# tensor4all/tensor4all-rs

Hardware: AMD Instinct MI355X
Metric: TCI2 full-sweep GF/s (d=30, chi=256 fp64) (higher is better)
Workload: dtype f64

## Files before the change

tensor4all-rs_amd/csrc/kernels.hpp:

```cpp
#pragma once

#include <hip/hip_runtime.h>

#include <cstddef>
#include <cstdint>

#include "../../include/t4a_testfunctions.h"

namespace t4a {

struct RrluWorkspace;

struct RrluPlan {
    int W = 1;
    int T = 256;
    int cpw = 0;
    int Mld = 0;
    size_t lds_bytes = 0;
};

RrluPlan rrlu_make_plan(int M, int N, int num_cus);

struct RrluArgs {
    const double* A;
// ... 160 lines not shown
size_t rrlu_xcd_cols_bytes(const RrluXcdPlan& plan, int M);
struct RrluXcdGroupArgs {
    RrluXcdArgs p[8];
};
void rrlu_xcd2_launch(const RrluXcdPlan& plan, const RrluXcdArgs& args, hipStream_t stream);
void rrlu_xcd2m_launch(const RrluXcdPlan& plan, const RrluXcdArgs& args, hipStream_t stream);
void rrlu_xcd2_group_launch(const RrluXcdPlan& plan, const RrluXcdGroupArgs& args, bool tie_row_major, hipStream_t stream);
bool rrlu_wg_make_plan(int M, int N, RrluXcdPlan* out, int spec_blocks = 0);
void rrlu_wg_launch(const RrluXcdPlan& plan, const RrluXcdArgs& args, hipStream_t stream);
void rrlu_wg_group_launch(const RrluXcdPlan& plan, const RrluXcdGroupArgs& args, bool tie_row_major, hipStream_t stream);
bool rrlu_w1_make_plan(int M, int N, RrluXcdPlan* out, int spec_blocks = 0);
void rrlu_w1_launch(const RrluXcdPlan& plan, const RrluXcdArgs& args, hipStream_t stream);
void rrlu_w1_group_launch(const RrluXcdPlan& plan, const RrluXcdGroupArgs& args, bool tie_row_major, hipStream_t stream);

void pi_eval_launch(const FnDevice& fn, const uint64_t* rowacc, int M, const uint64_t* colacc, int N, double* out,
                    int ld, bool transpose_out, unsigned long long* max_abs_bits, hipStream_t stream);
struct PiJob {
    const uint64_t* rowacc;
    const uint64_t* colacc;
    double* out;
    unsigned long long* max_abs_bits;
    int M, N, ld, pad_;
};
void pi_eval_batched_launch(const FnDevice& fn, const PiJob* d_jobs, int n_jobs, int max_M, int max_N, hipStream_t stream);
struct PackJob {
    const double* src;
    double* core;
    const int* info;
    int ld, L, S, R, last, pad_;
};
struct LuProblem;
constexpr int FILL_SMALL_MAX_N = 32, FILL_SMALL_MAX_RHS = 64;
void fill_small_launch(const FnDevice& fn, const PiJob* d_pis, const LuProblem* d_lups, const PackJob* d_packs, int n_jobs, int last_site,
                       hipStream_t stream);
void stage_copy_launch(const uint64_t* pinned_src, uint64_t* dst, size_t count, hipStream_t stream);
void absmax_launch(const double* data, size_t count, unsigned long long* max_abs_bits, hipStream_t stream);

constexpr int CHAIN_MAX_SET = 1024;
struct ChainTab {
    uint64_t* code;
    uint64_t* acc;
    int* cnt;
};
struct ChainCommon {
    ChainTab I, J, HI, HJ;
    ChainTab mI, mJ;
    int cap, K;
// ... 130 lines not shown

struct LuProblem {
    double* A; int lda; int n;
    int* piv;
    int* info;
    double* B; int ldb; int nrhs;
    const unsigned long long* pmax_bits;
};
void lu_batched_launch(const LuProblem* d_problems, int n_problems, int max_n, hipStream_t stream);
inline TrsmProblem lu_trsm_problem(const LuProblem& lp, bool lower, const int* skip_flag = nullptr)
{
    TrsmProblem t{};
    t.T = lp.A;
    t.ldt = lp.lda;
    t.n = lp.n;
    t.B = lp.B;
    t.ldb = lp.ldb;
    t.nrhs = lp.nrhs;
    t.lower = t.unit_diag = lower ? 1 : 0;
    t.skip_flag = skip_flag;
    return t;
}
constexpr int LU_MAX_PANEL_STEPS = 128;
bool lu_forward_blocked_launch(const LuProblem* d_problems, int n_problems, int max_n, int max_nrhs, hipStream_t stream, int avoid_xcc = -1,
                               unsigned* tickets = nullptr);
bool lu_solve_blocked_launch(const LuProblem* d_problems, int n_problems, int max_n, int max_nrhs, hipStream_t stream, int avoid_xcc = -1,
                             unsigned* tickets = nullptr);

void gather_launch(const double* in, int ldi, const int* rows, int nrows, const int* cols, int ncols, double* out,
                   int ldo, hipStream_t stream);
void scatter_rows_launch(const double* in, int ldi, const int* rows, int nrows, int ncols, double* out, int ldo,
                         hipStream_t stream);
void scatter_cols_launch(const double* in, int ldi, int nrows, const int* cols, int ncols, double* out, int ldo,
                         hipStream_t stream);
void fill_launch(double* p, size_t count, double value, hipStream_t stream);
void seq_matmul_launch(const double* A, int lda, const double* B, int ldb, double* C, int ldc, size_t M, size_t N, size_t K,
                       hipStream_t stream);
void set_identity_launch(double* p, int m, int n, int ld, hipStream_t stream);

struct TtCoreDesc { const double* data; int l, d, r; };
void tt_evaluate_launch(const TtCoreDesc* d_cores, int n_sites, int max_bond, const uint32_t* d_idx, int n_pts,
                        double* d_out, hipStream_t stream);


void core_reshape_launch(const double* in, int L, int S, int R, int mode, double* out, hipStream_t stream);
constexpr int PERMUTE_MAX_RANK = 16;
void permute_launch(const double* in, const size_t* dims, const size_t* perm, int rank, double* out, hipStream_t stream);
void tt_sum_launch(const TtCoreDesc* d_cores, int n_sites, int max_bond, double* d_out, hipStream_t stream);
enum : int {
    TT_SCALE_NONE = 0,
// ... 218 lines not shown
```

tensor4all-rs_amd/csrc/kernels_dense.hip:

```cpp
#include "kernels.hpp"

#include <algorithm>
#include <atomic>
#include <map>
#include <mutex>
#include <utility>
#include "common.hpp"

#include <cstdlib>

namespace t4a {

namespace {

typedef double double4_t __attribute__((ext_vector_type(4)));

constexpr int GBM = 64, GBK = 32, GPAD = 4;

template <int BN>
__global__ void __launch_bounds__(256) gemm_kernel(GemmDesc d)
{
    extern __shared__ __attribute__((aligned(16))) char gemm_smem[];
    typedef double TileA[GBK][GBM + GPAD];
    typedef double TileB[GBK][BN + GPAD];
// ... 625 lines not shown
#pragma unroll
    for (int r = 0; r < RP; ++r) {
        const int i = tid + 256 * r;
        if (i > J && i < m) {
            const double l = a[r][J] / piv;
            a[r][J] = l;
#pragma unroll
            for (int c = J + 1; c < NB; ++c) {
                const double prod = l * U[c];
                a[r][c] = a[r][c] - prod;
            }
        }
    }
}

template <int NB, int RP, int... Js>
__device__ __forceinline__ void lu_panel_columns(double (&a)[RP][NB], const PanelShared& sh, const LuProblem& pr, int kb, int m, int w, int tid,
                                                 int& first_bad, std::integer_sequence<int, Js...>)
{
    (lu_panel_column<NB, RP, Js>(a, sh, pr, kb, m, w, tid, first_bad), ...);
}

template <int NB, int RP>
__global__ void __launch_bounds__(256) lu_panel_kernel(const LuProblem* problems, int kb)
{
    __shared__ double U[2 * NB], V[2 * NB];
    __shared__ double red_v[8];
    __shared__ int red_i[8];
    const LuProblem pr = problems[blockIdx.x];
    const int n = pr.n;
    const int tid = threadIdx.x;
    if (kb == 0) {
        if (pr.pmax_bits) {
            const double pmax = __longlong_as_double((long long)*pr.pmax_bits);
            if (pmax < 2.220446049250313e-16) {
                if (tid == 0) pr.info[0] = -1;
                return;
            }
        }
        if (tid == 0) pr.info[0] = 0;
    } else if (pr.info[0] == -1) {
        return;
    }
    if (kb >= n) return;
    const int m = n - kb, w = (n - kb) < NB ? (n - kb) : NB;
    double* A = pr.A;
    const int lda = pr.lda;
    double a[RP][NB];
#pragma unroll
    for (int r = 0; r < RP; ++r) {
        const int i = tid + 256 * r;
#pragma unroll
        for (int c = 0; c < NB; ++c) a[r][c] = (i < m && c < w) ? A[(size_t)(kb + c) * lda + kb + i] : 0.0;
    }
    int first_bad = 0;
    PanelShared sh{U, V, red_v, red_i};
    lu_panel_columns<NB, RP>(a, sh, pr, kb, m, w, tid, first_bad, std::make_integer_sequence<int, NB>{});
    if (tid == 0 && first_bad != 0 && pr.info[0] == 0) pr.info[0] = first_bad;
#pragma unroll
    for (int r = 0; r < RP; ++r) {
        const int i = tid + 256 * r;
#pragma unroll
        for (int c = 0; c < NB; ++c)
            if (i < m && c < w) A[(size_t)(kb + c) * lda + kb + i] = a[r][c];
    }
}

__global__ void __launch_bounds__(256) lu_update_kernel(const LuProblem* problems, int kb, int nb, int tiles, int n_problems, int avoid_xcc,
                                                        unsigned* ticket, int a_only)
{
    extern __shared__ __attribute__((aligned(16))) char smem_raw[];
    __shared__ int s_item;
    if (avoid_xcc >= 0) {
        unsigned xcc;
        asm volatile("s_getreg_b32 %0, hwreg(HW_REG_XCC_ID)" : "=s"(xcc));
        if ((int)(xcc & 0xF) == avoid_xcc) return;
    }
    const int total_items = tiles * n_problems;
    bool first = true;
    for (;;) {
    __syncthreads();
    if (threadIdx.x == 0) s_item = ticket ? (int)atomicAdd(ticket, 1u) : (first ? (int)blockIdx.x : total_items);
    __syncthreads();
    first = false;
    const int item = s_item;
    if (item >= total_items) break;
    const LuProblem pr = problems[item / tiles];
    const int n = pr.n;
    if (kb >= n || pr.info[0] == -1) continue;
    const int ta = (n + nb - 1) / nb;
    const int nrhs = pr.B ? pr.nrhs : 0;
    const int t = item % tiles;
    const bool in_a = t < ta;
    const int c0 = in_a ? t * nb : (t - ta) * nb;
    if (!in_a && (a_only || c0 >= nrhs)) continue;
    if (in_a && c0 == kb) continue;
    const int m = n - kb, w = (n - kb) < nb ? (n - kb) : nb;
    const int lim = in_a ? n : nrhs;
    const int tc = (lim - c0) < nb ? (lim - c0) : nb;
    const bool left = in_a && c0 < kb;
// ... 104 lines not shown
{
    constexpr int ctrl = Q | (Q << 2) | (Q << 4) | (Q << 6);
    const long long b = __double_as_longlong(v);
    const int lo = __builtin_amdgcn_update_dpp(0, (int)(b & 0xFFFFFFFFll), ctrl, 0xF, 0xF, true);
    const int hi = __builtin_amdgcn_update_dpp(0, (int)(b >> 32), ctrl, 0xF, 0xF, true);
    return __longlong_as_double(((long long)hi << 32) | (unsigned int)lo);
}
template <int KK, bool LOWER> __device__ __forceinline__ void solve_block_step(double (&b)[4], const double (&dr)[SVB][4], const double (&rdr)[SVB], int g)
{
    constexpr int go = KK >> 2, to = KK & 3;
    double xk = quad_bcast_f64<go>(b[to]);
    if (!LOWER) xk = xk * rdr[KK];
    if (g == go) b[to] = xk;
#pragma unroll
    for (int t = 0; t < 4; ++t) b[t] = __builtin_fma(-dr[KK][t], xk, b[t]);
}
template <bool LOWER, int... KKs>
__device__ __forceinline__ void solve_block_steps(double (&b)[4], const double (&dr)[SVB][4], const double (&rdr)[SVB], int g, std::integer_sequence<int, KKs...>)
{
    if constexpr (LOWER) (solve_block_step<KKs, true>(b, dr, rdr, g), ...);
    else (solve_block_step<SVB - 1 - KKs, false>(b, dr, rdr, g), ...);
}

__global__ void __launch_bounds__(256) __attribute__((amdgpu_waves_per_eu(1, 1))) lu_solve_kernel(const LuProblem* problems, int cw, int n_problems, int chunks, int avoid_xcc, unsigned* ticket)
{
    extern __shared__ __attribute__((aligned(16))) char smem_raw[];
    __shared__ int s_item;
    if (avoid_xcc >= 0) {
        unsigned xcc;
        asm volatile("s_getreg_b32 %0, hwreg(HW_REG_XCC_ID)" : "=s"(xcc));
        if ((int)(xcc & 0xF) == avoid_xcc) return;
    }
    const int tid = threadIdx.x;
    const int lane = tid & 63, wave = tid >> 6;
    const int lr = lane & 15, lk = lane >> 4;
    const int cl = lane >> 2, g = lane & 3;
    const int total_items = chunks * n_problems;
    bool first = true;
    for (;;) {
        __syncthreads();
        if (tid == 0) s_item = ticket ? (int)atomicAdd(ticket, 1u) : (first ? (int)blockIdx.x : total_items);
        __syncthreads();
        first = false;
        const int item = s_item;
        if (item >= total_items) break;
        const LuProblem pr = problems[item / chunks];
        const int n = pr.n;
        const int c0 = (item % chunks) * cw;
        if (n <= 0 || !pr.B || c0 >= pr.nrhs || pr.info[0] == -1) continue;
        const int cwr = (pr.nrhs - c0) < cw ? (pr.nrhs - c0) : cw;
        const int ld = n | 1;
        double* Bs = reinterpret_cast<double*>(smem_raw);
        double* D = Bs + (size_t)ld * cw + ((ld * cw) & 1);
        double* rd = D + SVB * SVB;
        unsigned short* perm_s = reinterpret_cast<unsigned short*>(rd + SVB);
// ... 431 lines not shown
            hipLaunchKernelGGL(trsm_left_mfma_kernel, grid, dim3(256), lds, stream, d_problems, cw);
            return;
        }
    }
    int cw = (int)((128 * 1024) / ((size_t)max_n * 8));
    if (cw > 32) cw = 32;
    const long long total_cols = (long long)n_problems * max_nrhs;
    while (cw > 4 && total_cols / cw < 2048) cw /= 2;
    if (cw < 1) cw = 1;
    const size_t lds = (size_t)max_n * cw * 8;
    if (lds > 160 * 1024)
        throw Error(T4A_GPU_NOT_IMPLEMENTED, "triangular solve: systems with more than 20480 rows are not supported");
    dim3 grid((max_nrhs + cw - 1) / cw, n_problems);
    hipLaunchKernelGGL(trsm_left_kernel, grid, dim3(256), lds, stream, d_problems, cw);
}

void lu_batched_launch(const LuProblem* d_problems, int n_problems, int max_n, hipStream_t stream)
{
    if (n_problems <= 0) return;
    int T = max_n >= 128 ? 1024 : (max_n >= 32 ? 256 : 64);
    hipLaunchKernelGGL(lu_kernel, dim3(n_problems), dim3(T), 0, stream, d_problems);
}

bool lu_forward_blocked_launch(const LuProblem* d_problems, int n_problems, int max_n, int max_nrhs, hipStream_t stream, int avoid_xcc,
                               unsigned* tickets)
{
    if (n_problems <= 0 || max_n <= 0) return true;
    int nb;
    if (max_n <= 256) nb = 32;
    else if (max_n <= 512) nb = 16;
    else if (max_n <= 1024) nb = 8;
    else return false;
    static std::atomic<bool> attr_set{false};
    if (!attr_set) {
        (void)hipFuncSetAttribute(reinterpret_cast<const void*>(&lu_update_kernel),
                                  hipFuncAttributeMaxDynamicSharedMemorySize, 144 * 1024);
        (void)hipGetLastError();
        attr_set = true;
    }
    const int ldp = max_n | 1;
    const size_t lds_update = (size_t)ldp * nb * 8 * 2;
    const int tiles = (max_n + nb - 1) / nb + (max_nrhs + nb - 1) / nb + 1;
    for (int kb = 0; kb < max_n; kb += nb) {
        if (nb == 32) hipLaunchKernelGGL((lu_panel_kernel<32, 1>), dim3(n_problems), dim3(256), 0, stream, d_problems, kb);
        else if (nb == 16) hipLaunchKernelGGL((lu_panel_kernel<16, 2>), dim3(n_problems), dim3(256), 0, stream, d_problems, kb);
        else hipLaunchKernelGGL((lu_panel_kernel<8, 4>), dim3(n_problems), dim3(256), 0, stream, d_problems, kb);
        const int items = tiles * n_problems;
        unsigned* tk = tickets ? tickets + kb / nb : nullptr;
        const int grid = tk ? items + items / 7 + 8 : items;
        hipLaunchKernelGGL(lu_update_kernel, dim3(grid), dim3(256), lds_update, stream, d_problems, kb, nb, tiles, n_problems,
                           tk ? avoid_xcc : -1, tk, 0);
    }
    return true;
}

bool lu_solve_blocked_launch(const LuProblem* d_problems, int n_problems, int max_n, int max_nrhs, hipStream_t stream, int avoid_xcc,
                             unsigned* tickets)
{
    if (n_problems <= 0 || max_n <= 0) return true;
    if (max_n < 32 || max_n > 16 * 4 * SV_MAXS || max_nrhs < 16) return false;
    int nb;
    if (max_n <= 256) nb = 32;
    else nb = 16;
    static std::once_flag attr_once;
    std::call_once(attr_once, [] {
        (void)hipFuncSetAttribute(reinterpret_cast<const void*>(&lu_update_kernel), hipFuncAttributeMaxDynamicSharedMemorySize, 144 * 1024);
        (void)hipFuncSetAttribute(reinterpret_cast<const void*>(&lu_solve_kernel), hipFuncAttributeMaxDynamicSharedMemorySize, 160 * 1024);
        (void)hipGetLastError();
    });
    const int ldp = max_n | 1;
    const size_t lds_update = (size_t)ldp * nb * 8 * 2;
    const int tiles = (max_n + nb - 1) / nb;
    for (int kb = 0; kb < max_n; kb += nb) {
        if (nb == 32) hipLaunchKernelGGL((lu_panel_kernel<32, 1>), dim3(n_problems), dim3(256), 0, stream, d_problems, kb);
        else hipLaunchKernelGGL((lu_panel_kernel<16, 2>), dim3(n_problems), dim3(256), 0, stream, d_problems, kb);
        const int items = tiles * n_problems;
        unsigned* tk = tickets ? tickets + kb / nb : nullptr;
        const int grid = tk ? items + items / 7 + 8 : items;
        hipLaunchKernelGGL(lu_update_kernel, dim3(grid), dim3(256), lds_update, stream, d_problems, kb, nb, tiles, n_problems,
                           tk ? avoid_xcc : -1, tk, 1);
    }
    const size_t extra = (size_t)SVB * (SVB + 1) * 8 + SVB * 8 + 2 * (size_t)((max_n + 3) & ~3) * 2 + 64;
    int cw = 64;
    while (cw > 16 && (size_t)(max_n | 1) * cw * 8 + extra > 156 * 1024) cw -= 16;
    if (cw == 48) cw = 32;
    while (cw > 16 && max_nrhs <= cw / 2) cw /= 2;
    const size_t lds = (size_t)(max_n | 1) * cw * 8 + extra;
    const int chunks = (max_nrhs + cw - 1) / cw;
    const int items = chunks * n_problems;
    unsigned* tk = tickets ? tickets + (LU_MAX_PANEL_STEPS - 1) : nullptr;
    const int grid = tk ? items + items / 7 + 8 : items;
    hipLaunchKernelGGL(lu_solve_kernel, dim3(grid), dim3(256), lds, stream, d_problems, cw, n_problems, chunks, tk ? avoid_xcc : -1, tk);
    return true;
}

void tt_evaluate_launch(const TtCoreDesc* d_cores, int n_sites, int max_bond, const uint32_t* d_idx, int n_pts,
                        double* d_out, hipStream_t stream)
{
    if (n_pts <= 0) return;
    int blocks = n_pts < 4096 ? n_pts : 4096;
    const size_t lds = (size_t)2 * (max_bond > 0 ? max_bond : 1) * 8;
    hipLaunchKernelGGL(tt_eval_kernel, dim3(blocks), dim3(256), lds, stream, d_cores, n_sites, max_bond, d_idx, n_pts,
                       d_out);
}

}
```

tensor4all-rs_amd/csrc/kernels_pi.hip:

```cpp
#include "kernels.hpp"

namespace t4a {

namespace {

__device__ __forceinline__ void wave_absmax_commit(double av, unsigned long long* max_abs_bits)
{
#pragma unroll
    for (int off = 32; off >= 1; off >>= 1) {
        const double o = __shfl_xor(av, off);
        if (o > av) av = o;
    }
    if ((threadIdx.x & 63) == 0 && av > 0.0 && max_abs_bits)
        atomicMax(max_abs_bits, (unsigned long long)__double_as_longlong(av));
}

__global__ void __launch_bounds__(256) pi_eval_kernel(FnDevice fn, const uint64_t* __restrict__ rowacc, int M,
                                                      const uint64_t* __restrict__ colacc, int N,
                                                      double* __restrict__ out, int ld, int transpose_out,
                                                      unsigned long long* max_abs_bits)
{
    double av = 0.0;
    const int i = blockIdx.x * blockDim.x + threadIdx.x;
    uint64_t racc[T4A_FN_MAX_ACC] = {0, 0, 0, 0};
    if (i < M)
        for (int k = 0; k < fn.n_acc; ++k) racc[k] = rowacc[(size_t)i * fn.n_acc + k];
    for (int j = blockIdx.y; j < N; j += gridDim.y) {
        if (i < M) {
            uint64_t acc[T4A_FN_MAX_ACC] = {0, 0, 0, 0};
            for (int k = 0; k < fn.n_acc; ++k) acc[k] = racc[k] + colacc[(size_t)j * fn.n_acc + k];
            const double v = t4a_fn_value(fn.fid, acc, fn.params);
            if (transpose_out)
                out[(size_t)i * ld + j] = v;
            else
                out[(size_t)j * ld + i] = v;
            const double a = sqrt(v * v);
            if (a > av) av = a;
        }
    }
    wave_absmax_commit(av, max_abs_bits);
}

__global__ void __launch_bounds__(256) pi_eval_batched_kernel(FnDevice fn, const PiJob* __restrict__ jobs)
{
    const PiJob jb = jobs[blockIdx.z];
    double av = 0.0;
    const int i = blockIdx.x * blockDim.x + threadIdx.x;
    if (blockIdx.x * (int)blockDim.x >= jb.M) return;
    uint64_t racc[T4A_FN_MAX_ACC] = {0, 0, 0, 0};
    if (i < jb.M)
        for (int k = 0; k < fn.n_acc; ++k) racc[k] = jb.rowacc[(size_t)i * fn.n_acc + k];
    for (int j = blockIdx.y; j < jb.N; j += gridDim.y) {
        if (i < jb.M) {
            uint64_t acc[T4A_FN_MAX_ACC] = {0, 0, 0, 0};
            for (int k = 0; k < fn.n_acc; ++k) acc[k] = racc[k] + jb.colacc[(size_t)j * fn.n_acc + k];
            const double v = t4a_fn_value(fn.fid, acc, fn.params);
            jb.out[(size_t)j * jb.ld + i] = v;
            const double a = sqrt(v * v);
            if (a > av) av = a;
        }
    }
    wave_absmax_commit(av, jb.max_abs_bits);
}

__global__ void __launch_bounds__(256) absmax_kernel(const double* __restrict__ data, size_t count,
                                                     unsigned long long* max_abs_bits)
{
    double av = 0.0;
    for (size_t i = (size_t)blockIdx.x * blockDim.x + threadIdx.x; i < count; i += (size_t)gridDim.x * blockDim.x) {
        const double v = data[i];
        const double a = sqrt(v * v);
        if (a > av) av = a;
    }
    wave_absmax_commit(av, max_abs_bits);
}

__global__ void __launch_bounds__(256) stage_copy_kernel(const uint64_t* __restrict__ src, uint64_t* __restrict__ dst, size_t count)
{
    for (size_t i = (size_t)blockIdx.x * blockDim.x + threadIdx.x; i < count; i += (size_t)gridDim.x * blockDim.x) dst[i] = src[i];
}

}

void stage_copy_launch(const uint64_t* pinned_src, uint64_t* dst, size_t count, hipStream_t stream)
{
    if (count == 0) return;
    size_t blocks = (count + 255) / 256;
    if (blocks > 64) blocks = 64;
    hipLaunchKernelGGL(stage_copy_kernel, dim3((unsigned)blocks), dim3(256), 0, stream, pinned_src, dst, count);
}

void pi_eval_launch(const FnDevice& fn, const uint64_t* rowacc, int M, const uint64_t* colacc, int N, double* out,
                    int ld, bool transpose_out, unsigned long long* max_abs_bits, hipStream_t stream)
{
    if (M <= 0 || N <= 0) return;
    dim3 block(256);
    int gy = N < 2048 ? N : 2048;
    dim3 grid((M + 255) / 256, gy);
    hipLaunchKernelGGL(pi_eval_kernel, grid, block, 0, stream, fn, rowacc, M, colacc, N, out, ld,
                       transpose_out ? 1 : 0, max_abs_bits);
}

void pi_eval_batched_launch(const FnDevice& fn, const PiJob* d_jobs, int n_jobs, int max_M, int max_N, hipStream_t stream)
{
    if (n_jobs <= 0 || max_M <= 0 || max_N <= 0) return;
    const int gy = max_N < 512 ? max_N : 512;
    dim3 grid((max_M + 255) / 256, gy, n_jobs);
    hipLaunchKernelGGL(pi_eval_batched_kernel, grid, dim3(256), 0, stream, fn, d_jobs);
}

namespace {

struct FillSmallArgs {
    FnDevice fn;
    const PiJob* pis;
    const LuProblem* lups;
    const PackJob* packs;
    int n_jobs, last_site;
};

__global__ void __launch_bounds__(256) fill_small_kernel(FillSmallArgs a)
{
    __shared__ double As[FILL_SMALL_MAX_N * FILL_SMALL_MAX_N];
    __shared__ double Bs[FILL_SMALL_MAX_N * FILL_SMALL_MAX_RHS];
    __shared__ double red_v[4];
    __shared__ int red_i[4];
    __shared__ int piv_s, info_s;
    __shared__ double pivval_s;
    const int k = blockIdx.x, tid = threadIdx.x, T = blockDim.x, lane = tid & 63, wave = tid >> 6;
    if (k >= a.n_jobs) return;
// ... 167 lines not shown
```

tensor4all-rs_amd/csrc/tci2.hpp:

```cpp
#pragma once

#include <cstring>
#include <memory>
#include <vector>

#include "engine.hpp"
#include "fnsource.hpp"
#include "matrix_source.hpp"
#include "stdrng.hpp"
#include "pishard.hpp"
#include "rook.hpp"
#include "tt.hpp"

namespace t4a {

struct TCI2Options {
    double tolerance = 1e-8;
    size_t max_iter = 20;
    size_t max_bond_dim = 0;
    int pivot_search = 0;
    bool normalize_error = true;
    size_t verbosity = 0;
    size_t max_nglobal_pivot = 5;
    size_t nsearch = 5;
// ... 14 lines not shown
};

struct FillZero {
    double* ptr;
    size_t count;
};
struct FillOps {
    void* flags;
    size_t flag_bytes;
    void* stage_dev;
    const void* stage_host;
    size_t stage_bytes;
    const PiJob* pis;
    const LuProblem* lups;
    const TrsmProblem* trs;
    const PackJob* packs;
    unsigned* tickets;
    const int* info_dev;
    int* info_host;
    size_t info_bytes;
    FnDevice fn;
    int n_pi, max_M, max_N;
    int n_lu, max_n, max_nrhs;
    int avoid_xcc;
    unsigned pack_gx, pack_gy;
    int n_site_jobs, last_site;
    int small;
};
static_assert(sizeof(FillOps) == 13 * 8 + sizeof(FnDevice) + 12 * 4 && sizeof(FnDevice) == 8 + 8 * T4A_FN_MAX_PARAMS, "no padding: compared bytewise");
struct FillRecords {
    std::vector<FillZero> zeros;
    FillOps ops{};
    bool operator==(const FillRecords& o) const
    {
        return zeros.size() == o.zeros.size() && std::memcmp(&ops, &o.ops, sizeof(FillOps)) == 0 &&
               (zeros.empty() || std::memcmp(zeros.data(), o.zeros.data(), zeros.size() * sizeof(FillZero)) == 0);
    }
};
struct FillOptions {
    bool async = false;
    bool trust_cache = false;
    bool no_main_sync = false;
};

class Tci2 {
    pool::IdleScope idle_scope_;
public:
    explicit Tci2(const std::vector<size_t>& local_dims);
    ~Tci2();

    void set_builtin(int fid, int n_acc, const double* params, const uint64_t* weights);
    void set_callback(t4a_gpu_batch_eval_fn cb, void* ctx);
// ... 119 lines not shown
        size_t bond = 0;
        bool cols = false;
        IndexSet set;
        std::vector<uint64_t> acc;
    };
    SidePrep prep_;
    struct Prefetch {
        bool wanted = false;
        size_t bond = 0;
        bool cols = false;
        const IndexSet* extra = nullptr;
        long fill_site = -1;
    } prefetch_;
    struct FillAcc {
        bool valid = false;
        std::vector<uint64_t> accJ, accK, accI;
    };
    struct FillState {
        std::vector<FillAcc> cache;
        DevBuf<double> A, B;
        DevBuf<int> piv;
        DevBuf<unsigned long long> flags;
        PinBuf<int> hinfo;
        PinBuf<uint64_t> hstage;
        DevBuf<uint64_t> dstage;
        std::vector<size_t> solved_sites;
        EventTimer ev;
        hipStream_t stream = nullptr, import_stream = nullptr;
        hipEvent_t export_event = nullptr, import_event = nullptr;
        bool inflight = false, timed = false, import_inflight = false;
        bool cores_shared_async = false;
        bool cores_shared_legacy_stream = false;
        uint64_t stats[3] = {0, 0, 0};
        FillRecords last, graph;
        hipGraphExec_t graph_exec = nullptr;
        bool graph_broken = false;
    } fill_;
    void fill_run(FillOptions opt);
    void fill_presize(const TCI2Options& options);
    void issue_fill_ops(const FillRecords& rec);
    void export_cores_async(size_t first, size_t step, double* d_dst, size_t stride, hipStream_t consumer, const char* what);
    void prepare_fill_site(size_t b);
    void invalidate_fill_cache();
    void build_side(size_t bond, bool cols, const IndexSet& extra, SidePrep& out) const;
    LuciResult luci_on_sets(const IndexSet& is, const IndexSet& js, const RrLUOptions& o, bool need_factors,
                            const std::vector<uint64_t>* acc_rows = nullptr, const std::vector<uint64_t>* acc_cols = nullptr);
// ... 105 lines not shown
```

tensor4all-rs_amd/csrc/tci2_fill.hip:

```cpp
#include "tci2.hpp"

#include <algorithm>
#include <atomic>
#include <chrono>
#include <cstdio>
#include <cstdlib>
#include <cstring>
#include <exception>
#include <string>

namespace t4a {

namespace {

__global__ void __launch_bounds__(256) pack_fill_batched_kernel(const PackJob* __restrict__ jobs)
{
    const PackJob j = jobs[blockIdx.y];
    const size_t total = (size_t)j.L * j.S * j.R;
    const bool zero = j.info && *j.info == -1;
    for (size_t e = (size_t)blockIdx.x * blockDim.x + threadIdx.x; e < total; e += (size_t)gridDim.x * blockDim.x) {
        const int l = (int)(e % j.L);
        const int s = (int)((e / j.L) % j.S);
        const int r = (int)(e / ((size_t)j.L * j.S));
        if (j.last)
            j.core[e] = j.src[(size_t)r * j.ld + (l * j.S + s)];
        else
            j.core[e] = zero ? 0.0 : j.src[(size_t)(l * j.S + s) * j.ld + r];
    }
}

enum : unsigned { FILL_ZEROS = 1, FILL_FLAGS = 2, FILL_SOLVE = 4, FILL_ALL = 7 };

void fill_issue(const FillRecords& rec, unsigned parts, hipStream_t st)
{
    const FillOps& o = rec.ops;
    if (parts & FILL_ZEROS)
        for (const FillZero& z : rec.zeros) fill_launch(z.ptr, z.count, 0.0, st);
    if (parts & FILL_FLAGS) T4A_HIP(hipMemsetAsync(o.flags, 0, o.flag_bytes, st));
    if (!(parts & FILL_SOLVE)) return;
    T4A_HIP(hipMemcpyAsync(o.stage_dev, o.stage_host, o.stage_bytes, hipMemcpyHostToDevice, st));
    if (o.small) {
        fill_small_launch(o.fn, o.pis, o.lups, o.packs, o.n_site_jobs, o.last_site, st);
        T4A_HIP(hipMemcpyAsync(o.info_host, o.info_dev, o.info_bytes, hipMemcpyDeviceToHost, st));
        return;
    }
    if (o.n_pi) pi_eval_batched_launch(o.fn, o.pis, o.n_pi, o.max_M, o.max_N, st);
    if (o.n_lu) {
        if (!lu_solve_blocked_launch(o.lups, o.n_lu, o.max_n, o.max_nrhs, st, o.avoid_xcc, o.tickets)) {
            if (!lu_forward_blocked_launch(o.lups, o.n_lu, o.max_n, o.max_nrhs, st, o.avoid_xcc, o.tickets)) {
                lu_batched_launch(o.lups, o.n_lu, o.max_n, st);
                trsm_left_batched_launch(o.trs, o.n_lu, o.max_n, o.max_nrhs, st);
            }
            trsm_left_batched_launch(o.trs + o.n_lu, o.n_lu, o.max_n, o.max_nrhs, st);
        }
    }
    hipLaunchKernelGGL(pack_fill_batched_kernel, dim3(o.pack_gx, o.pack_gy), dim3(256), 0, st, o.packs);
    T4A_HIP(hipMemcpyAsync(o.info_host, o.info_dev, o.info_bytes, hipMemcpyDeviceToHost, st));
}

struct SiteJob {
    size_t b;
    size_t ni, nj, np;
    size_t offA, offB;
    double *A, *B;
    unsigned long long* pmax;
    size_t accJ, accK, accI;
    bool last;
};
struct FillTables {
    std::vector<LuProblem> lups;
    std::vector<TrsmProblem> trl, tru;
    std::vector<PackJob> packs;
// ... 132 lines not shown
    std::vector<size_t> lb(n_ + 1, 1), rb(n_ + 1, 1);
    for (size_t b = 0; b < n_; ++b) lb[b + 1] = std::min(chi, lb[b] * local_dims[b]);
    for (size_t b = n_; b-- > 0;) rb[b] = std::min(chi, rb[b + 1] * local_dims[b]);
    auto bond = [&](size_t b) { return std::min(lb[b], rb[b]); };
    auto mine = [&](size_t b) { return shard_world <= 1 || (b % shard_world) == shard_rank; };
    size_t totA = 0, totB = 0, tot_cores = 0, acc_words = 0;
    for (size_t b = 0; b < n_; ++b) {
        if (!mine(b)) continue;
        const size_t l = bond(b), rr = bond(b + 1);
        tot_cores += l * local_dims[b] * rr;
        totA += rr * rr;
        totB += rr * l * local_dims[b];
        acc_words += chi * (2 + local_dims[b]) * (size_t)fn_.dev.n_acc;
    }
    if ((tot_cores + totA + totB) * sizeof(double) > ((size_t)1 << 30)) return;
    for (size_t b = 0; b < n_; ++b)
        if (mine(b)) cores[b].buf.reserve(std::max<size_t>(bond(b) * local_dims[b] * bond(b + 1), 1));
    fill_.A.reserve(std::max<size_t>(totA, 1));
    fill_.B.reserve(std::max<size_t>(totB, 1));
    fill_.piv.reserve(std::max<size_t>(n_ * chi, 1));
    const size_t desc_bytes = n_ * (2 * sizeof(PiJob) + sizeof(LuProblem) + 2 * sizeof(TrsmProblem) + 64) + 256;
    fill_.hstage.reserve(acc_words + desc_bytes / 8 + 64);
    fill_.dstage.reserve(acc_words + desc_bytes / 8 + 64);
    fill_.flags.reserve(n_ + (n_ + 1) / 2 + (LU_MAX_PANEL_STEPS + 1) / 2);
    fill_.hinfo.reserve(n_);
}

void Tci2::fill_site_tensors() { fill_run(FillOptions()); }

void Tci2::issue_fill_ops(const FillRecords& rec)
{
    hipStream_t st = fill_.stream;
    static const bool use_graph = std::getenv("T4A_NO_FILL_GRAPH") == nullptr;
    if (fill_.timed) T4A_HIP(hipEventRecord(fill_.ev.a, st));
    bool done = false;
    const bool shared_ok = !fill_.cores_shared_async || (fill_graph_relaxed && !fill_.cores_shared_legacy_stream);
    if (use_graph && !fill_.graph_broken && shared_ok) {
        if (fill_.graph_exec && rec == fill_.graph) {
            T4A_HIP(hipGraphLaunch(fill_.graph_exec, st));
            ++fill_.stats[1];
            done = true;
        } else if (rec == fill_.last) {
            if (fill_.graph_exec) {
                (void)hipGraphExecDestroy(fill_.graph_exec);
                fill_.graph_exec = nullptr;
            }
            hipGraph_t graph = nullptr;
            pool::capture_begin();
            bool ok = hipStreamBeginCapture(st, hipStreamCaptureModeThreadLocal) == hipSuccess;
            if (ok) {
                try {
                    fill_issue(rec, FILL_ALL, st);
                } catch (...) {
                    ok = false;
                }
                if (hipStreamEndCapture(st, &graph) != hipSuccess || !graph) ok = false;
            }
            pool::capture_end();
            if (ok && hipGraphInstantiate(&fill_.graph_exec, graph, nullptr, nullptr, 0) != hipSuccess) {
                fill_.graph_exec = nullptr;
                ok = false;
            }
            if (graph) (void)hipGraphDestroy(graph);
            if (ok) {
                fill_.graph = rec;
                T4A_HIP(hipGraphLaunch(fill_.graph_exec, st));
                ++fill_.stats[2];
                done = true;
            } else {
                (void)hipGetLastError();
                fill_.graph_broken = true;
            }
        }
    }
    fill_.last = rec;
    ++fill_.stats[0];
    if (!done) fill_issue(rec, FILL_ALL, st);
    if (fill_.timed) T4A_HIP(hipEventRecord(fill_.ev.b, st));
}

void Tci2::fill_wait()
{
    if (fill_.import_inflight) {
        fill_.import_inflight = false;
        T4A_HIP(hipStreamSynchronize(fill_.import_stream));
    }
    if (!fill_.inflight) return;
    fill_.inflight = false;
    T4A_HIP(hipStreamSynchronize(fill_.stream));
    T4A_HIP(hipGetLastError());
    if (eng.prof.enabled && fill_.timed) {
        float ms = 0.f;
        T4A_HIP(hipEventElapsedTime(&ms, fill_.ev.a, fill_.ev.b));
        eng.prof.v[4] += ms;
        eng.prof.v[5] += 1.0;
    }
    fill_.timed = false;
    for (size_t k = 0; k < fill_.solved_sites.size(); ++k)
        if (fill_.hinfo.get()[fill_.solved_sites[k]] > 0) {
            const size_t site = fill_.solved_sites[k];
            fill_.solved_sites.clear();
            throw Error(T4A_GPU_INTERNAL_ERROR, "one-site interpolation solve failed: singular pivot matrix at site " +
                                                    std::to_string(site));
        }
    fill_.solved_sites.clear();
}

void Tci2::fill_run(FillOptions opt)
{
    fn_.require("tci2");
    HostLap lap;
    if (!opt.trust_cache) invalidate_fill_cache();
    const bool builtin = fn_.builtin();
    if (!builtin) sync_digits();
    fill_wait();
    if (!fill_.stream) fill_.stream = pool::stream_get(2);
    static const bool sync_fill = std::getenv("T4A_SYNC_FILL") != nullptr;
    if (!builtin || sync_fill) opt.async = false;
    const bool no_main_sync = opt.no_main_sync && builtin;
    if (!no_main_sync) T4A_HIP(hipStreamSynchronize(eng.stream()));
// ... 20 lines not shown
        j.nj = nj;
        j.last = (b == n_ - 1);
        j.np = j.last ? 0 : i_set[b + 1].count;
        if (!j.last && j.np != nj)
            throw Error(T4A_GPU_INTERNAL_ERROR, "one-site interpolation solve failed: pivot matrix at bond " +
                                                    std::to_string(b) + " is not square (" + std::to_string(j.np) + " x " +
                                                    std::to_string(nj) + ")");
        j.offA = totA;
        j.offB = totB;
        j.accJ = j.accK = j.accI = 0;
        totA += j.last ? 0 : nj * j.np;
        totB += nj * ni;
        jobs.push_back(j);
    }
    lap(g_prof.wait_jobs);
    if (jobs.empty()) {
        fill_issue(rec, FILL_ZEROS, st);
        T4A_HIP(hipStreamSynchronize(st));
        return;
    }
    if (!builtin) fill_issue(rec, FILL_ZEROS, st);
    fill_.A.reserve(std::max<size_t>(totA, 1));
    fill_.B.reserve(totB);
    const size_t fm_words = n_ + (n_ + 1) / 2 + (LU_MAX_PANEL_STEPS + 1) / 2;
    fill_.flags.reserve(fm_words);
    unsigned long long* d_max = fill_.flags.get();
    int* d_info = reinterpret_cast<int*>(fill_.flags.get() + n_);
    fill_.hinfo.reserve(n_);
    ops.flags = fill_.flags.get();
    ops.flag_bytes = fm_words * sizeof(unsigned long long);
    ops.tickets = reinterpret_cast<unsigned*>(fill_.flags.get() + n_ + (n_ + 1) / 2);
    ops.avoid_xcc = (no_main_sync && !xcd_disabled()) ? eng.xcc() : -1;
    ops.info_dev = d_info;
    ops.info_host = fill_.hinfo.get();
    ops.info_bytes = n_ * sizeof(int);
    ops.fn = fn_.dev;
    fill_.timed = eng.prof.enabled;
    if (!builtin) {
        if (fill_.timed) T4A_HIP(hipEventRecord(fill_.ev.a, st));
        fill_issue(rec, FILL_FLAGS, st);
        T4A_HIP(hipStreamSynchronize(st));
    }

    size_t piv_total = 0;
    for (SiteJob& j : jobs) {
        j.A = j.last ? nullptr : fill_.A.get() + j.offA;
        j.B = fill_.B.get() + j.offB;
        j.pmax = d_max + j.b;
        DevCore& c = cores[j.b];
        c.reshape((j.b == 0) ? 1 : i_set[j.b].count, local_dims[j.b], j.last ? 1 : j.np);
        piv_total += j.np;
    }
    fill_.piv.reserve(std::max<size_t>(piv_total, 1));

    FillTables tab;
    size_t piv_off = 0, max_core = 1;
    fill_.solved_sites.clear();
    double flops = 0.0;
// ... 63 lines not shown
            }
            eng.prof.v[11] += (double)j.ni * j.nj + (double)j.np * j.nj;
        }
        invalidate_fill_cache();
        lap(g_prof.accumulators);
    } else {
        for (const SiteJob& j : jobs) {
            IndexSet ik = kronecker_i(j.b);
            const IndexSet& jb = j_set[j.b];
            if (j.last) {
                eval_matrix(ik, 0, jb, ik.width, j.B, nullptr);
            } else {
                eval_matrix(jb, j.b + 1, ik, 0, j.B, nullptr);
                eval_matrix(jb, j.b + 1, i_set[j.b + 1], 0, j.A, j.pmax);
            }
        }
        T4A_HIP(hipStreamSynchronize(eng.stream()));
        acc_used_ = 0;
        lap(g_prof.staging);
    }
    fill_stage(fill_.hstage, fill_.dstage, jobs, acc_all, builtin, tab, ops, lap);
    lap(g_prof.staging);
    eng.prof.v[10] += flops;
    if (!builtin) {
        fill_issue(rec, FILL_SOLVE, st);
        if (fill_.timed) T4A_HIP(hipEventRecord(fill_.ev.b, st));
    } else {
        issue_fill_ops(rec);
    }
    fill_.inflight = true;
    if (g_prof.on) {
        g_prof.total += std::chrono::duration<double, std::micro>(std::chrono::steady_clock::now() - lap.t0).count();
        lap(g_prof.issue);
        const HostProfile& p = g_prof;
        if (++g_prof.calls % 20 == 0) {
            const double c = (double)p.calls;
            std::fprintf(stderr, "[host profile] fill_site_tensors host part %.1f us per call (wait+jobs %.1f, descriptors %.1f, "
                                 "accumulators %.1f, staging %.1f, issue %.1f)\n",
                         p.total / c, p.wait_jobs / c, p.descriptors / c, p.accumulators / c, p.staging / c, p.issue / c);
            std::fprintf(stderr, "[host profile]   staging in detail: reserve %.1f, accumulator copy %.1f, job tables %.1f us per call\n",
                         p.reserve / c, p.acc_copy / c, p.job_tables / c);
        }
    }
    if (!opt.async) fill_wait();
}

// ... 92 lines not shown
```

Baseline: 342.3.

## Keep pi-eval and LU panel kernels off the bond-chain XCD via ticket scheduling

Extends XCD avoidance, previously applied only to the LU update and solve kernels, to the batched pi evaluation and the LU panel kernels. Each gets a persistent ticket-based variant whose workgroups exit when they land on avoided XCDs, with the remaining workgroups pulling items atomically. Ticket counters are copied back to the host and compared with the expected item counts; if any work was left untaken, the fill is reissued without avoidance and avoidance is switched off for the process. The pi ticket kernel reserves a large LDS allocation and the panel kernel sets waves_per_eu, presumably to control occupancy and placement. This adds atomic overhead and a validation step.

Result: no change. 343.7 (median of 6 runs) (+0.4%).

```diff
diff --git a/tensor4all-rs_amd/csrc/kernels.hpp b/tensor4all-rs_amd/csrc/kernels.hpp
--- a/tensor4all-rs_amd/csrc/kernels.hpp
+++ b/tensor4all-rs_amd/csrc/kernels.hpp
@@ -206,7 +206,8 @@
     unsigned long long* max_abs_bits;
     int M, N, ld, pad_;
 };
-void pi_eval_batched_launch(const FnDevice& fn, const PiJob* d_jobs, int n_jobs, int max_M, int max_N, hipStream_t stream);
+void pi_eval_batched_launch(const FnDevice& fn, const PiJob* d_jobs, int n_jobs, int max_M, int max_N, hipStream_t stream,
+                            unsigned avoid_mask = 0, unsigned* ticket = nullptr, unsigned* expect = nullptr);
 struct PackJob {
     const double* src;
     double* core;
@@ -383,10 +384,21 @@
     return t;
 }
 constexpr int LU_MAX_PANEL_STEPS = 128;
-bool lu_forward_blocked_launch(const LuProblem* d_problems, int n_problems, int max_n, int max_nrhs, hipStream_t stream, int avoid_xcc = -1,
-                               unsigned* tickets = nullptr);
-bool lu_solve_blocked_launch(const LuProblem* d_problems, int n_problems, int max_n, int max_nrhs, hipStream_t stream, int avoid_xcc = -1,
-                             unsigned* tickets = nullptr);
+constexpr int LU_TICKETS = 2 * LU_MAX_PANEL_STEPS;
+inline int ticket_grid(int items) { return items + items / 7 + 8; }
+#ifdef __HIPCC__
+__device__ __forceinline__ bool on_avoided_xcd(unsigned avoid_mask)
+{
+    if (!avoid_mask) return false;
+    unsigned xcc;
+    asm volatile("s_getreg_b32 %0, hwreg(HW_REG_XCC_ID)" : "=s"(xcc));
+    return (avoid_mask >> (xcc & 0xF)) & 1u;
+}
+#endif
+bool lu_forward_blocked_launch(const LuProblem* d_problems, int n_problems, int max_n, int max_nrhs, hipStream_t stream, unsigned avoid_mask = 0,
+                               unsigned* tickets = nullptr, unsigned* expect = nullptr);
+bool lu_solve_blocked_launch(const LuProblem* d_problems, int n_problems, int max_n, int max_nrhs, hipStream_t stream, unsigned avoid_mask = 0,
+                             unsigned* tickets = nullptr, unsigned* expect = nullptr);
 
 void gather_launch(const double* in, int ldi, const int* rows, int nrows, const int* cols, int ncols, double* out,
                    int ldo, hipStream_t stream);
diff --git a/tensor4all-rs_amd/csrc/kernels_dense.hip b/tensor4all-rs_amd/csrc/kernels_dense.hip
--- a/tensor4all-rs_amd/csrc/kernels_dense.hip
+++ b/tensor4all-rs_amd/csrc/kernels_dense.hip
@@ -671,14 +671,9 @@
 }
 
 template <int NB, int RP>
-__global__ void __launch_bounds__(256) lu_panel_kernel(const LuProblem* problems, int kb)
-{
-    __shared__ double U[2 * NB], V[2 * NB];
-    __shared__ double red_v[8];
-    __shared__ int red_i[8];
-    const LuProblem pr = problems[blockIdx.x];
+__device__ __forceinline__ void lu_panel_problem(const LuProblem& pr, int kb, const PanelShared& sh, const int tid)
+{
     const int n = pr.n;
-    const int tid = threadIdx.x;
     if (kb == 0) {
         if (pr.pmax_bits) {
             const double pmax = __longlong_as_double((long long)*pr.pmax_bits);
@@ -703,7 +698,6 @@
         for (int c = 0; c < NB; ++c) a[r][c] = (i < m && c < w) ? A[(size_t)(kb + c) * lda + kb + i] : 0.0;
     }
     int first_bad = 0;
-    PanelShared sh{U, V, red_v, red_i};
     lu_panel_columns<NB, RP>(a, sh, pr, kb, m, w, tid, first_bad, std::make_integer_sequence<int, NB>{});
     if (tid == 0 && first_bad != 0 && pr.info[0] == 0) pr.info[0] = first_bad;
 #pragma unroll
@@ -715,16 +709,44 @@
     }
 }
 
-__global__ void __launch_bounds__(256) lu_update_kernel(const LuProblem* problems, int kb, int nb, int tiles, int n_problems, int avoid_xcc,
+template <int NB, int RP>
+__global__ void __launch_bounds__(256) lu_panel_kernel(const LuProblem* problems, int kb)
+{
+    __shared__ double U[2 * NB], V[2 * NB];
+    __shared__ double red_v[8];
+    __shared__ int red_i[8];
+    const LuProblem pr = problems[blockIdx.x];
+    lu_panel_problem<NB, RP>(pr, kb, PanelShared{U, V, red_v, red_i}, threadIdx.x);
+}
+
+template <int NB, int RP>
+__global__ void __launch_bounds__(256) __attribute__((amdgpu_waves_per_eu(5))) lu_panel_ticket_kernel(const LuProblem* problems, int kb, int n_problems, unsigned avoid_mask,
+                                                              unsigned* ticket)
+{
+    __shared__ double U[2 * NB], V[2 * NB];
+    __shared__ double red_v[8];
+    __shared__ int red_i[8];
+    __shared__ int s_item;
+    if (on_avoided_xcd(avoid_mask)) return;
+    for (;;) {
+        __syncthreads();
+        if (threadIdx.x == 0) s_item = (int)atomicAdd(ticket, 1u);
+        __syncthreads();
+        const int item = __builtin_amdgcn_readfirstlane(s_item);
+        if (item >= n_problems) break;
+        const LuProblem pr = problems[item];
+        int tid = threadIdx.x;
+        asm volatile("" : "+v"(tid));
+        lu_panel_problem<NB, RP>(pr, kb, PanelShared{U, V, red_v, red_i}, tid);
+    }
+}
+
+__global__ void __launch_bounds__(256) lu_update_kernel(const LuProblem* problems, int kb, int nb, int tiles, int n_problems, unsigned avoid_mask,
                                                         unsigned* ticket, int a_only)
 {
     extern __shared__ __attribute__((aligned(16))) char smem_raw[];
     __shared__ int s_item;
-    if (avoid_xcc >= 0) {
-        unsigned xcc;
-        asm volatile("s_getreg_b32 %0, hwreg(HW_REG_XCC_ID)" : "=s"(xcc));
-        if ((int)(xcc & 0xF) == avoid_xcc) return;
-    }
+    if (on_avoided_xcd(avoid_mask)) return;
     const int total_items = tiles * n_problems;
     bool first = true;
     for (;;) {
@@ -875,15 +897,11 @@
     else (solve_block_step<SVB - 1 - KKs, false>(b, dr, rdr, g), ...);
 }
 
-__global__ void __launch_bounds__(256) __attribute__((amdgpu_waves_per_eu(1, 1))) lu_solve_kernel(const LuProblem* problems, int cw, int n_problems, int chunks, int avoid_xcc, unsigned* ticket)
+__global__ void __launch_bounds__(256) __attribute__((amdgpu_waves_per_eu(1, 1))) lu_solve_kernel(const LuProblem* problems, int cw, int n_problems, int chunks, unsigned avoid_mask, unsigned* ticket)
 {
     extern __shared__ __attribute__((aligned(16))) char smem_raw[];
     __shared__ int s_item;
-    if (avoid_xcc >= 0) {
-        unsigned xcc;
-        asm volatile("s_getreg_b32 %0, hwreg(HW_REG_XCC_ID)" : "=s"(xcc));
-        if ((int)(xcc & 0xF) == avoid_xcc) return;
-    }
+    if (on_avoided_xcd(avoid_mask)) return;
     const int tid = threadIdx.x;
     const int lane = tid & 63, wave = tid >> 6;
     const int lr = lane & 15, lk = lane >> 4;
@@ -1361,8 +1379,32 @@
     hipLaunchKernelGGL(lu_kernel, dim3(n_problems), dim3(T), 0, stream, d_problems);
 }
 
-bool lu_forward_blocked_launch(const LuProblem* d_problems, int n_problems, int max_n, int max_nrhs, hipStream_t stream, int avoid_xcc,
-                               unsigned* tickets)
+namespace {
+template <int NB, int RP>
+void lu_panel_launch(const LuProblem* d_problems, int n_problems, int kb, hipStream_t stream, unsigned avoid_mask, unsigned* ticket, unsigned* expect)
+{
+    if (ticket && avoid_mask) {
+        if (expect) *expect = (unsigned)n_problems;
+        hipLaunchKernelGGL((lu_panel_ticket_kernel<NB, RP>), dim3(ticket_grid(n_problems)), dim3(256), 0, stream, d_problems, kb, n_problems,
+                           avoid_mask, ticket);
+    } else {
+        hipLaunchKernelGGL((lu_panel_kernel<NB, RP>), dim3(n_problems), dim3(256), 0, stream, d_problems, kb);
+    }
+}
+void lu_panel_launch(int nb, const LuProblem* d_problems, int n_problems, int kb, hipStream_t stream, unsigned avoid_mask, unsigned* tickets,
+                     unsigned* expect)
+{
+    const int k = LU_MAX_PANEL_STEPS + kb / nb;
+    unsigned* tk = tickets ? tickets + k : nullptr;
+    unsigned* ex = expect ? expect + k : nullptr;
+    if (nb == 32) lu_panel_launch<32, 1>(d_problems, n_problems, kb, stream, avoid_mask, tk, ex);
+    else if (nb == 16) lu_panel_launch<16, 2>(d_problems, n_problems, kb, stream, avoid_mask, tk, ex);
+    else lu_panel_launch<8, 4>(d_problems, n_problems, kb, stream, avoid_mask, tk, ex);
+}
+}
+
+bool lu_forward_blocked_launch(const LuProblem* d_problems, int n_problems, int max_n, int max_nrhs, hipStream_t stream, unsigned avoid_mask,
+                               unsigned* tickets, unsigned* expect)
 {
     if (n_problems <= 0 || max_n <= 0) return true;
     int nb;
@@ -1381,20 +1423,19 @@
     const size_t lds_update = (size_t)ldp * nb * 8 * 2;
     const int tiles = (max_n + nb - 1) / nb + (max_nrhs + nb - 1) / nb + 1;
     for (int kb = 0; kb < max_n; kb += nb) {
-        if (nb == 32) hipLaunchKernelGGL((lu_panel_kernel<32, 1>), dim3(n_problems), dim3(256), 0, stream, d_problems, kb);
-        else if (nb == 16) hipLaunchKernelGGL((lu_panel_kernel<16, 2>), dim3(n_problems), dim3(256), 0, stream, d_problems, kb);
-        else hipLaunchKernelGGL((lu_panel_kernel<8, 4>), dim3(n_problems), dim3(256), 0, stream, d_problems, kb);
+        lu_panel_launch(nb, d_problems, n_problems, kb, stream, avoid_mask, tickets, expect);
         const int items = tiles * n_problems;
         unsigned* tk = tickets ? tickets + kb / nb : nullptr;
-        const int grid = tk ? items + items / 7 + 8 : items;
+        const int grid = tk ? ticket_grid(items) : items;
+        if (tk && expect) expect[kb / nb] = (unsigned)items;
         hipLaunchKernelGGL(lu_update_kernel, dim3(grid), dim3(256), lds_update, stream, d_problems, kb, nb, tiles, n_problems,
-                           tk ? avoid_xcc : -1, tk, 0);
+                           tk ? avoid_mask : 0u, tk, 0);
     }
     return true;
 }
 
-bool lu_solve_blocked_launch(const LuProblem* d_problems, int n_problems, int max_n, int max_nrhs, hipStream_t stream, int avoid_xcc,
-                             unsigned* tickets)
+bool lu_solve_blocked_launch(const LuProblem* d_problems, int n_problems, int max_n, int max_nrhs, hipStream_t stream, unsigned avoid_mask,
+                             unsigned* tickets, unsigned* expect)
 {
     if (n_problems <= 0 || max_n <= 0) return true;
     if (max_n < 32 || max_n > 16 * 4 * SV_MAXS || max_nrhs < 16) return false;
@@ -1411,13 +1452,13 @@
     const size_t lds_update = (size_t)ldp * nb * 8 * 2;
     const int tiles = (max_n + nb - 1) / nb;
     for (int kb = 0; kb < max_n; kb += nb) {
-        if (nb == 32) hipLaunchKernelGGL((lu_panel_kernel<32, 1>), dim3(n_problems), dim3(256), 0, stream, d_problems, kb);
-        else hipLaunchKernelGGL((lu_panel_kernel<16, 2>), dim3(n_problems), dim3(256), 0, stream, d_problems, kb);
+        lu_panel_launch(nb, d_problems, n_problems, kb, stream, avoid_mask, tickets, expect);
         const int items = tiles * n_problems;
         unsigned* tk = tickets ? tickets + kb / nb : nullptr;
-        const int grid = tk ? items + items / 7 + 8 : items;
+        const int grid = tk ? ticket_grid(items) : items;
+        if (tk && expect) expect[kb / nb] = (unsigned)items;
         hipLaunchKernelGGL(lu_update_kernel, dim3(grid), dim3(256), lds_update, stream, d_problems, kb, nb, tiles, n_problems,
-                           tk ? avoid_xcc : -1, tk, 1);
+                           tk ? avoid_mask : 0u, tk, 1);
     }
     const size_t extra = (size_t)SVB * (SVB + 1) * 8 + SVB * 8 + 2 * (size_t)((max_n + 3) & ~3) * 2 + 64;
     int cw = 64;
@@ -1428,8 +1469,9 @@
     const int chunks = (max_nrhs + cw - 1) / cw;
     const int items = chunks * n_problems;
     unsigned* tk = tickets ? tickets + (LU_MAX_PANEL_STEPS - 1) : nullptr;
-    const int grid = tk ? items + items / 7 + 8 : items;
-    hipLaunchKernelGGL(lu_solve_kernel, dim3(grid), dim3(256), lds, stream, d_problems, cw, n_problems, chunks, tk ? avoid_xcc : -1, tk);
+    const int grid = tk ? ticket_grid(items) : items;
+    if (tk && expect) expect[LU_MAX_PANEL_STEPS - 1] = (unsigned)items;
+    hipLaunchKernelGGL(lu_solve_kernel, dim3(grid), dim3(256), lds, stream, d_problems, cw, n_problems, chunks, tk ? avoid_mask : 0u, tk);
     return true;
 }
 
diff --git a/tensor4all-rs_amd/csrc/kernels_pi.hip b/tensor4all-rs_amd/csrc/kernels_pi.hip
--- a/tensor4all-rs_amd/csrc/kernels_pi.hip
+++ b/tensor4all-rs_amd/csrc/kernels_pi.hip
@@ -41,16 +41,15 @@
     wave_absmax_commit(av, max_abs_bits);
 }
 
-__global__ void __launch_bounds__(256) pi_eval_batched_kernel(FnDevice fn, const PiJob* __restrict__ jobs)
-{
-    const PiJob jb = jobs[blockIdx.z];
+__device__ __forceinline__ void pi_eval_item(const FnDevice& fn, const PiJob& jb, int bx, int by, int stripes)
+{
     double av = 0.0;
-    const int i = blockIdx.x * blockDim.x + threadIdx.x;
-    if (blockIdx.x * (int)blockDim.x >= jb.M) return;
+    const int i = bx * (int)blockDim.x + threadIdx.x;
+    if (bx * (int)blockDim.x >= jb.M) return;
     uint64_t racc[T4A_FN_MAX_ACC] = {0, 0, 0, 0};
     if (i < jb.M)
         for (int k = 0; k < fn.n_acc; ++k) racc[k] = jb.rowacc[(size_t)i * fn.n_acc + k];
-    for (int j = blockIdx.y; j < jb.N; j += gridDim.y) {
+    for (int j = by; j < jb.N; j += stripes) {
         if (i < jb.M) {
             uint64_t acc[T4A_FN_MAX_ACC] = {0, 0, 0, 0};
             for (int k = 0; k < fn.n_acc; ++k) acc[k] = racc[k] + jb.colacc[(size_t)j * fn.n_acc + k];
@@ -63,6 +62,31 @@
     wave_absmax_commit(av, jb.max_abs_bits);
 }
 
+__global__ void __launch_bounds__(256) pi_eval_batched_kernel(FnDevice fn, const PiJob* __restrict__ jobs)
+{
+    const PiJob jb = jobs[blockIdx.z];
+    pi_eval_item(fn, jb, blockIdx.x, blockIdx.y, gridDim.y);
+}
+
+constexpr unsigned PI_TICKET_LDS = 56 * 1024;
+constexpr int PI_TICKET_STRIPES = 128;
+__global__ void __launch_bounds__(256) pi_eval_batched_ticket_kernel(FnDevice fn, const PiJob* __restrict__ jobs, int gx, int gy, int n_jobs,
+                                                                     unsigned avoid_mask, unsigned* ticket)
+{
+    __shared__ int s_item;
+    if (on_avoided_xcd(avoid_mask)) return;
+    const int total_items = gx * gy * n_jobs;
+    for (;;) {
+        __syncthreads();
+        if (threadIdx.x == 0) s_item = (int)atomicAdd(ticket, 1u);
+        __syncthreads();
+        const int item = __builtin_amdgcn_readfirstlane(s_item);
+        if (item >= total_items) break;
+        const PiJob jb = jobs[item / (gx * gy)];
+        pi_eval_item(fn, jb, (item / gy) % gx, item % gy, gy);
+    }
+}
+
 __global__ void __launch_bounds__(256) absmax_kernel(const double* __restrict__ data, size_t count,
                                                      unsigned long long* max_abs_bits)
 {
@@ -101,11 +125,21 @@
                        transpose_out ? 1 : 0, max_abs_bits);
 }
 
-void pi_eval_batched_launch(const FnDevice& fn, const PiJob* d_jobs, int n_jobs, int max_M, int max_N, hipStream_t stream)
+void pi_eval_batched_launch(const FnDevice& fn, const PiJob* d_jobs, int n_jobs, int max_M, int max_N, hipStream_t stream, unsigned avoid_mask,
+                            unsigned* ticket, unsigned* expect)
 {
     if (n_jobs <= 0 || max_M <= 0 || max_N <= 0) return;
     const int gy = max_N < 512 ? max_N : 512;
-    dim3 grid((max_M + 255) / 256, gy, n_jobs);
+    const int gx = (max_M + 255) / 256;
+    const int gy_t = max_N < PI_TICKET_STRIPES ? max_N : PI_TICKET_STRIPES;
+    const long long items = (long long)gx * gy_t * n_jobs;
+    if (ticket && avoid_mask && items < (1ll << 30)) {
+        if (expect) *expect = (unsigned)items;
+        hipLaunchKernelGGL(pi_eval_batched_ticket_kernel, dim3(ticket_grid((int)items)), dim3(256), PI_TICKET_LDS, stream, fn, d_jobs, gx, gy_t,
+                           n_jobs, avoid_mask, ticket);
+        return;
+    }
+    dim3 grid(gx, gy, n_jobs);
     hipLaunchKernelGGL(pi_eval_batched_kernel, grid, dim3(256), 0, stream, fn, d_jobs);
 }
 
diff --git a/tensor4all-rs_amd/csrc/tci2.hpp b/tensor4all-rs_amd/csrc/tci2.hpp
--- a/tensor4all-rs_amd/csrc/tci2.hpp
+++ b/tensor4all-rs_amd/csrc/tci2.hpp
@@ -60,12 +60,13 @@
     FnDevice fn;
     int n_pi, max_M, max_N;
     int n_lu, max_n, max_nrhs;
-    int avoid_xcc;
+    unsigned avoid_mask;
     unsigned pack_gx, pack_gy;
     int n_site_jobs, last_site;
     int small;
 };
 static_assert(sizeof(FillOps) == 13 * 8 + sizeof(FnDevice) + 12 * 4 && sizeof(FnDevice) == 8 + 8 * T4A_FN_MAX_PARAMS, "no padding: compared bytewise");
+constexpr int FILL_TICKET_PI = LU_TICKETS, FILL_TICKETS = LU_TICKETS + 2;
 struct FillRecords {
     std::vector<FillZero> zeros;
     FillOps ops{};
@@ -231,6 +232,8 @@
         DevBuf<int> piv;
         DevBuf<unsigned long long> flags;
         PinBuf<int> hinfo;
+        std::vector<unsigned> expect, graph_expect;
+        bool avoiding = false;
         PinBuf<uint64_t> hstage;
         DevBuf<uint64_t> dstage;
         std::vector<size_t> solved_sites;
diff --git a/tensor4all-rs_amd/csrc/tci2_fill.hip b/tensor4all-rs_amd/csrc/tci2_fill.hip
--- a/tensor4all-rs_amd/csrc/tci2_fill.hip
+++ b/tensor4all-rs_amd/csrc/tci2_fill.hip
@@ -29,11 +29,14 @@
     }
 }
 
+std::atomic<bool> g_fill_avoid_off{false};
+
 enum : unsigned { FILL_ZEROS = 1, FILL_FLAGS = 2, FILL_SOLVE = 4, FILL_ALL = 7 };
 
-void fill_issue(const FillRecords& rec, unsigned parts, hipStream_t st)
+void fill_issue(const FillRecords& rec, unsigned parts, hipStream_t st, unsigned* expect = nullptr)
 {
     const FillOps& o = rec.ops;
+    if (expect) std::fill(expect, expect + FILL_TICKETS, 0u);
     if (parts & FILL_ZEROS)
         for (const FillZero& z : rec.zeros) fill_launch(z.ptr, z.count, 0.0, st);
     if (parts & FILL_FLAGS) T4A_HIP(hipMemsetAsync(o.flags, 0, o.flag_bytes, st));
@@ -44,10 +47,12 @@
         T4A_HIP(hipMemcpyAsync(o.info_host, o.info_dev, o.info_bytes, hipMemcpyDeviceToHost, st));
         return;
     }
-    if (o.n_pi) pi_eval_batched_launch(o.fn, o.pis, o.n_pi, o.max_M, o.max_N, st);
+    if (o.n_pi)
+        pi_eval_batched_launch(o.fn, o.pis, o.n_pi, o.max_M, o.max_N, st, o.avoid_mask, o.tickets + FILL_TICKET_PI,
+                               expect ? expect + FILL_TICKET_PI : nullptr);
     if (o.n_lu) {
-        if (!lu_solve_blocked_launch(o.lups, o.n_lu, o.max_n, o.max_nrhs, st, o.avoid_xcc, o.tickets)) {
-            if (!lu_forward_blocked_launch(o.lups, o.n_lu, o.max_n, o.max_nrhs, st, o.avoid_xcc, o.tickets)) {
+        if (!lu_solve_blocked_launch(o.lups, o.n_lu, o.max_n, o.max_nrhs, st, o.avoid_mask, o.tickets, expect)) {
+            if (!lu_forward_blocked_launch(o.lups, o.n_lu, o.max_n, o.max_nrhs, st, o.avoid_mask, o.tickets, expect)) {
                 lu_batched_launch(o.lups, o.n_lu, o.max_n, st);
                 trsm_left_batched_launch(o.trs, o.n_lu, o.max_n, o.max_nrhs, st);
             }
@@ -226,8 +231,8 @@
     const size_t desc_bytes = n_ * (2 * sizeof(PiJob) + sizeof(LuProblem) + 2 * sizeof(TrsmProblem) + 64) + 256;
     fill_.hstage.reserve(acc_words + desc_bytes / 8 + 64);
     fill_.dstage.reserve(acc_words + desc_bytes / 8 + 64);
-    fill_.flags.reserve(n_ + (n_ + 1) / 2 + (LU_MAX_PANEL_STEPS + 1) / 2);
-    fill_.hinfo.reserve(n_);
+    fill_.flags.reserve(n_ + (n_ + 1) / 2 + FILL_TICKETS / 2);
+    fill_.hinfo.reserve((n_ + 1) / 2 * 2 + FILL_TICKETS);
 }
 
 void Tci2::fill_site_tensors() { fill_run(FillOptions()); }
@@ -235,6 +240,7 @@
 void Tci2::issue_fill_ops(const FillRecords& rec)
 {
     hipStream_t st = fill_.stream;
+    fill_.expect.resize(FILL_TICKETS);
     static const bool use_graph = std::getenv("T4A_NO_FILL_GRAPH") == nullptr;
     if (fill_.timed) T4A_HIP(hipEventRecord(fill_.ev.a, st));
     bool done = false;
@@ -242,6 +248,7 @@
     if (use_graph && !fill_.graph_broken && shared_ok) {
         if (fill_.graph_exec && rec == fill_.graph) {
             T4A_HIP(hipGraphLaunch(fill_.graph_exec, st));
+            fill_.expect = fill_.graph_expect;
             ++fill_.stats[1];
             done = true;
         } else if (rec == fill_.last) {
@@ -254,7 +261,7 @@
             bool ok = hipStreamBeginCapture(st, hipStreamCaptureModeThreadLocal) == hipSuccess;
             if (ok) {
                 try {
-                    fill_issue(rec, FILL_ALL, st);
+                    fill_issue(rec, FILL_ALL, st, fill_.expect.data());
                 } catch (...) {
                     ok = false;
                 }
@@ -268,6 +275,7 @@
             if (graph) (void)hipGraphDestroy(graph);
             if (ok) {
                 fill_.graph = rec;
+                fill_.graph_expect = fill_.expect;
                 T4A_HIP(hipGraphLaunch(fill_.graph_exec, st));
                 ++fill_.stats[2];
                 done = true;
@@ -279,7 +287,8 @@
     }
     fill_.last = rec;
     ++fill_.stats[0];
-    if (!done) fill_issue(rec, FILL_ALL, st);
+    if (!done) fill_issue(rec, FILL_ALL, st, fill_.expect.data());
+    fill_.avoiding = rec.ops.avoid_mask != 0;
     if (fill_.timed) T4A_HIP(hipEventRecord(fill_.ev.b, st));
 }
 
@@ -300,6 +309,22 @@
         eng.prof.v[5] += 1.0;
     }
     fill_.timed = false;
+    if (fill_.avoiding) {
+        fill_.avoiding = false;
+        const unsigned* tk = reinterpret_cast<const unsigned*>(fill_.hinfo.get() + (n_ + 1) / 2 * 2);
+        bool short_of = false;
+        for (int i = 0; i < FILL_TICKETS; ++i) short_of = short_of || tk[i] < fill_.expect[i];
+        if (short_of) {
+            if (!g_fill_avoid_off.exchange(true, std::memory_order_relaxed))
+                std::fprintf(stderr, "[t4a] fill_site_tensors no longer keeps off the bond chain's XCD in this process (workgroup placement "
+                                     "did not hold: work items of a fill were left untaken); the fill is issued again\n");
+            FillRecords again = fill_.last;
+            again.ops.avoid_mask = 0;
+            fill_issue(again, FILL_ALL, fill_.stream);
+            T4A_HIP(hipStreamSynchronize(fill_.stream));
+            T4A_HIP(hipGetLastError());
+        }
+    }
     for (size_t k = 0; k < fill_.solved_sites.size(); ++k)
         if (fill_.hinfo.get()[fill_.solved_sites[k]] > 0) {
             const size_t site = fill_.solved_sites[k];
@@ -366,18 +391,24 @@
     if (!builtin) fill_issue(rec, FILL_ZEROS, st);
     fill_.A.reserve(std::max<size_t>(totA, 1));
     fill_.B.reserve(totB);
-    const size_t fm_words = n_ + (n_ + 1) / 2 + (LU_MAX_PANEL_STEPS + 1) / 2;
+    static_assert(FILL_TICKETS % 2 == 0, "whole words");
+    const size_t fm_words = n_ + (n_ + 1) / 2 + FILL_TICKETS / 2;
     fill_.flags.reserve(fm_words);
     unsigned long long* d_max = fill_.flags.get();
     int* d_info = reinterpret_cast<int*>(fill_.flags.get() + n_);
-    fill_.hinfo.reserve(n_);
+    fill_.hinfo.reserve((n_ + 1) / 2 * 2 + FILL_TICKETS);
     ops.flags = fill_.flags.get();
     ops.flag_bytes = fm_words * sizeof(unsigned long long);
     ops.tickets = reinterpret_cast<unsigned*>(fill_.flags.get() + n_ + (n_ + 1) / 2);
-    ops.avoid_xcc = (no_main_sync && !xcd_disabled()) ? eng.xcc() : -1;
+    const bool avoid = no_main_sync && !xcd_disabled() && !g_fill_avoid_off.load(std::memory_order_relaxed) && eng.xcc() >= 0 && eng.xcc() < 16;
+    ops.avoid_mask = avoid ? 1u << eng.xcc() : 0u;
+#ifdef T4A_TEST_HOOKS
+    if (const char* m = std::getenv("T4A_TEST_FILL_AVOID"))
+        ops.avoid_mask = (builtin && !g_fill_avoid_off.load(std::memory_order_relaxed)) ? (unsigned)std::atoi(m) & 0xFFFFu : 0u;
+#endif
     ops.info_dev = d_info;
     ops.info_host = fill_.hinfo.get();
-    ops.info_bytes = n_ * sizeof(int);
+    ops.info_bytes = ((n_ + 1) / 2 * 2 + FILL_TICKETS) * sizeof(int);
     ops.fn = fn_.dev;
     fill_.timed = eng.prof.enabled;
     if (!builtin) {
@@ -487,6 +518,11 @@
     fill_stage(fill_.hstage, fill_.dstage, jobs, acc_all, builtin, tab, ops, lap);
     lap(g_prof.staging);
     eng.prof.v[10] += flops;
+#ifdef T4A_TEST_HOOKS
+    if (std::getenv("T4A_TEST_FILL_TRACE"))
+        std::fprintf(stderr, "[t4a test] fill avoid_mask=%u small=%d n_pi=%d n_lu=%d beside_chain=%d\n", ops.avoid_mask, ops.small, ops.n_pi, ops.n_lu,
+                     no_main_sync ? 1 : 0);
+#endif
     if (!builtin) {
         fill_issue(rec, FILL_SOLVE, st);
         if (fill_.timed) T4A_HIP(hipEventRecord(fill_.ev.b, st));
```
